# tyiannak/pyAudioAnalysis

Hardware: AMD Instinct MI355X
Metric: short-term frames/sec (34-feat, 16 kHz, 50 ms/25 ms) + HBM GB/s vs peak (higher is better)
Workload: dtype f64

## Files before the change

### include/paa_hip.h

```cpp
#ifndef PAA_HIP_H
#define PAA_HIP_H

#include <stddef.h>
#include <stdint.h>

#ifdef __cplusplus
extern "C" {
#endif

#define PAA_OK                 0
#define PAA_ERR_ARG          (-1)
#define PAA_ERR_UNSUPPORTED  (-2)
#define PAA_ERR_HIP          (-3)
#define PAA_ERR_OOM          (-4)
#define PAA_ERR_TOO_SHORT    (-5)
#define PAA_ERR_CHROMA_VALUE (-6)
#define PAA_ERR_CHROMA_INDEX (-7)
#define PAA_ERR_MEL_INDEX    (-8)
#define PAA_ERR_COMM         (-9)

#define PAA_N_BASE_FEATURES 34

const char *paa_version(void);
const char *paa_last_error(void);
// ... 133 lines not shown
                           const int64_t *offsets, int64_t n_seq, int32_t *d_states, double *d_logprob);
int paa_hmm_dev_loglik_f64(const void *handle, const double *d_feats, int n_dims, int64_t ld, int64_t n_vec, double *d_loglik);
int paa_hmm_train_stats_f64(const double *feats, int n_dims, int64_t ld, int64_t n_vec, const int32_t *labels, int n_states,
                            double *priors, double *transmat, double *means, double *covars);
int paa_hmm_dev_train_stats_f64(const double *d_feats, int n_dims, int64_t ld, int64_t n_vec, const int32_t *labels,
                                int n_states, double *priors, double *transmat, double *means, double *covars);
int paa_debug_hmm_dev_decode_f64(const void *handle, const double *d_feats, int n_dims, int64_t ld, int64_t n_vec,
                                 const int64_t *offsets, int64_t n_seq, int32_t *d_states, double *d_logprob,
                                 int64_t block_rows);

int paa_diar_dev_standardize_f64(const double *d_feats, int n_dims, int64_t ld, int64_t n_vec, double *d_z, double *stats);
int paa_diar_dev_select_rows_f64(const double *d_z, int n_dims, int64_t ld, int64_t n_vec, const int32_t *rows, int n_rows,
                                 double *d_out);
int paa_diar_dev_dim_distances_f64(const double *d_z, int n_dims, int64_t ld, int64_t n_vec, const int32_t *d_labels,
                                   const int32_t *ks, int nk, double *colsum, double *pair_mean);
int paa_diar_dev_sqdist_points_f64(const double *d_z, int n_dims, int64_t ld, int64_t n_vec, const int64_t *idx, int n_pts,
                                   double *out);
int paa_diar_dev_get_points_f64(const double *d_z, int n_dims, int64_t ld, int64_t n_vec, const int64_t *idx, int n_pts,
                                double *out);
int paa_diar_dev_kmeans_f64(const double *d_z, int n_dims, int64_t ld, int64_t n_vec, const int32_t *ks, int nk, double *centers,
                            double tol, int max_iter, int32_t *d_labels, int32_t *n_iter, double *inertia);
int paa_diar_dev_pair_sums_f64(const double *d_z, int n_dims, int64_t ld, int64_t n_vec, const int32_t *d_labels,
                               const int32_t *ks, int nk, double *sums);

int paa_lda_dev_class_stats_f64(const double *d_x, int n_dims, int64_t ld, int64_t n_vec, const int64_t *run_offsets,
                                int64_t n_classes, double *means, double *within_std);
int paa_lda_dev_within_gram_f64(const double *d_x, int n_dims, int64_t ld, int64_t n_vec, const int64_t *run_offsets,
                                int64_t n_classes, const double *means, const double *within_std, double fac, double *gram);
int paa_lda_dev_project_f64(const double *d_x, int n_dims, int64_t ld, int64_t n_vec, const double *xbar, const double *scalings,
                            int n_out, double *d_y, int64_t ld_y);

#define PAA_COMM_ID_BYTES 128
int paa_comm_unique_id(void *id_out );
int paa_comm_init(int world_size, int rank, const void *id);
int paa_comm_destroy(void);
int paa_comm_gather_f64(const double *d_send, const int64_t *counts, int root, double *d_recv);
int paa_comm_gatherv_f64(const double *d_send, const int64_t *counts, const int64_t *displs, int root, double *d_recv);
int paa_comm_barrier(void);

int paa_debug_mel_bank(double fs, int num_fft, double *out_dense);
int paa_debug_dct(double *out_13x40);
int paa_debug_chroma(double fs, int num_fft, int capacity, int32_t *src, double *weight, int32_t *slot);
int paa_debug_wave_trace(uint64_t *out, int max_waves);
int paa_debug_lane_peak(void);
int paa_debug_phase_cycles(uint64_t *out16);
int paa_debug_fft_plan(int window, int32_t *radices, int32_t *fft_len);
int paa_debug_comm_marker_name(const void *unique_id, int rank, char *out, int capacity);
int paa_debug_tri_plan(int window, double fs, int32_t *shape8, int32_t *offsets6, unsigned char *blob, int capacity);
int paa_debug_wg_plan(int window, int32_t *info32, uint16_t *perm, int perm_capacity);
int paa_debug_wgs_plan(int window, int32_t *info16, int32_t *bin_of, int capacity);
int paa_debug_wgr_tables(double fs, int window, int32_t *mel_job, int32_t *mel_fil, int32_t *ch_n, int32_t *ch_src, double *ch_w);
int paa_debug_wgr_runs(const int64_t *frames, int64_t n_clips, int num_cu, int32_t *runs3, int64_t capacity, int64_t *n_runs);
int paa_debug_blu_plan(int window, double fs, int32_t *info8, int32_t *offsets3, unsigned char *blob, int capacity);
int paa_debug_lane_jobs(const int32_t *first, const int32_t *wfirst, const int32_t *cnt, int n_owners, int32_t *jobs256);
int paa_debug_mix_plan(int window, int32_t *radices, int32_t *fft_len, uint16_t *perm, int perm_capacity,
                       int32_t *waves, int32_t *tw_global);
int paa_debug_run_plan(const int64_t *frames, int64_t n_clips, int quantum, int min_run, int max_run, int halo, int wg_runs,
                       int num_cu, int32_t *run_cap, int64_t *n_runs, int32_t *longest);
int paa_debug_run_plan_shrink(const int64_t *frames, int64_t n_clips, int quantum, int min_run, int max_run, int shrink,
                              int wg_runs, int num_cu, int32_t *run_cap, int64_t *n_runs, int32_t *longest);
int64_t paa_debug_balanced_runs(const int64_t *frames, int64_t n_clips, int run_cap, int quantum, int shrink, int wg_runs,
                                int num_cu, int min_run, int32_t *lens, int64_t capacity);

#ifdef __cplusplus
}
#endif
#endif
```

### pyaudioanalysis_amd/_ffi.py

```python
import ctypes as C
import os
import threading

import numpy as np

from . import _build

PAA_OK = 0
ERR_ARG, ERR_UNSUPPORTED, ERR_HIP, ERR_OOM = -1, -2, -3, -4
ERR_TOO_SHORT, ERR_CHROMA_VALUE, ERR_CHROMA_INDEX, ERR_MEL_INDEX, ERR_COMM = -5, -6, -7, -8, -9
COMM_ID_BYTES = 128

_lock = threading.Lock()
_lib = None

c_i16p = C.POINTER(C.c_int16)
c_f64p = C.POINTER(C.c_double)
c_i64p = C.POINTER(C.c_int64)
c_i32p = C.POINTER(C.c_int32)


class HipLibraryError(RuntimeError):
    """libpaa_hip.so is missing / unbuildable, or the HIP runtime reported an error."""

# ... 86 lines not shown
    "paa_forest_destroy": (C.c_int, [C.c_void_p]),
    "paa_forest_num_classes": (C.c_int, [C.c_void_p]),
    "paa_forest_predict_f64": (C.c_int, [C.c_void_p, c_f64p, C.c_int, C.c_int64, C.c_int64, c_f64p, c_f64p, c_i32p, c_f64p,
                                         c_f64p]),
    "paa_forest_dev_predict_f64": (C.c_int, [C.c_void_p, C.c_void_p, C.c_int, C.c_int64, C.c_int64, C.c_void_p, C.c_void_p,
                                             C.c_void_p, C.c_void_p, C.c_void_p]),
    "paa_hmm_create": (C.c_int, [c_f64p, c_f64p, c_f64p, c_f64p, C.c_int, C.c_int, C.POINTER(C.c_void_p)]),
    "paa_hmm_destroy": (C.c_int, [C.c_void_p]),
    "paa_hmm_num_states": (C.c_int, [C.c_void_p]),
    "paa_hmm_decode_f64": (C.c_int, [C.c_void_p, c_f64p, C.c_int, C.c_int64, C.c_int64, c_i64p, C.c_int64, c_i32p, c_f64p]),
    "paa_hmm_dev_decode_f64": (C.c_int, [C.c_void_p, C.c_void_p, C.c_int, C.c_int64, C.c_int64, c_i64p, C.c_int64, C.c_void_p,
                                         C.c_void_p]),
    "paa_hmm_dev_loglik_f64": (C.c_int, [C.c_void_p, C.c_void_p, C.c_int, C.c_int64, C.c_int64, C.c_void_p]),
    "paa_hmm_train_stats_f64": (C.c_int, [c_f64p, C.c_int, C.c_int64, C.c_int64, c_i32p, C.c_int, c_f64p, c_f64p, c_f64p,
                                          c_f64p]),
    "paa_hmm_dev_train_stats_f64": (C.c_int, [C.c_void_p, C.c_int, C.c_int64, C.c_int64, c_i32p, C.c_int, c_f64p, c_f64p,
                                              c_f64p, c_f64p]),
    "paa_debug_hmm_dev_decode_f64": (C.c_int, [C.c_void_p, C.c_void_p, C.c_int, C.c_int64, C.c_int64, c_i64p, C.c_int64,
                                               C.c_void_p, C.c_void_p, C.c_int64]),
    "paa_diar_dev_standardize_f64": (C.c_int, [C.c_void_p, C.c_int, C.c_int64, C.c_int64, C.c_void_p, c_f64p]),
    "paa_diar_dev_select_rows_f64": (C.c_int, [C.c_void_p, C.c_int, C.c_int64, C.c_int64, c_i32p, C.c_int, C.c_void_p]),
    "paa_diar_dev_dim_distances_f64": (C.c_int, [C.c_void_p, C.c_int, C.c_int64, C.c_int64, C.c_void_p, c_i32p, C.c_int, c_f64p,
                                                 c_f64p]),
    "paa_diar_dev_sqdist_points_f64": (C.c_int, [C.c_void_p, C.c_int, C.c_int64, C.c_int64, c_i64p, C.c_int, c_f64p]),
    "paa_diar_dev_get_points_f64": (C.c_int, [C.c_void_p, C.c_int, C.c_int64, C.c_int64, c_i64p, C.c_int, c_f64p]),
    "paa_diar_dev_kmeans_f64": (C.c_int, [C.c_void_p, C.c_int, C.c_int64, C.c_int64, c_i32p, C.c_int, c_f64p, C.c_double,
                                          C.c_int, C.c_void_p, c_i32p, c_f64p]),
    "paa_diar_dev_pair_sums_f64": (C.c_int, [C.c_void_p, C.c_int, C.c_int64, C.c_int64, C.c_void_p, c_i32p, C.c_int, c_f64p]),
    "paa_lda_dev_class_stats_f64": (C.c_int, [C.c_void_p, C.c_int, C.c_int64, C.c_int64, c_i64p, C.c_int64, c_f64p, c_f64p]),
    "paa_lda_dev_within_gram_f64": (C.c_int, [C.c_void_p, C.c_int, C.c_int64, C.c_int64, c_i64p, C.c_int64, c_f64p, c_f64p,
                                              C.c_double, c_f64p]),
    "paa_lda_dev_project_f64": (C.c_int, [C.c_void_p, C.c_int, C.c_int64, C.c_int64, c_f64p, c_f64p, C.c_int, C.c_void_p,
                                          C.c_int64]),
    "paa_comm_unique_id": (C.c_int, [C.c_void_p]),
    "paa_comm_init": (C.c_int, [C.c_int, C.c_int, C.c_void_p]),
    "paa_comm_destroy": (C.c_int, []),
    "paa_comm_gather_f64": (C.c_int, [C.c_void_p, c_i64p, C.c_int, C.c_void_p]),
    "paa_comm_gatherv_f64": (C.c_int, [C.c_void_p, c_i64p, c_i64p, C.c_int, C.c_void_p]),
    "paa_comm_barrier": (C.c_int, []),
    "paa_debug_mel_bank": (C.c_int, [C.c_double, C.c_int, c_f64p]),
    "paa_debug_dct": (C.c_int, [c_f64p]),
    "paa_debug_chroma": (C.c_int, [C.c_double, C.c_int, C.c_int, c_i32p, c_f64p, c_i32p]),
    "paa_debug_phase_cycles": (C.c_int, [C.POINTER(C.c_uint64)]),
    "paa_debug_wave_trace": (C.c_int, [C.POINTER(C.c_uint64), C.c_int]),
    "paa_debug_lane_peak": (C.c_int, []),
    "paa_debug_fft_plan": (C.c_int, [C.c_int, c_i32p, c_i32p]),
    "paa_debug_comm_marker_name": (C.c_int, [C.c_void_p, C.c_int, C.c_char_p, C.c_int]),
    "paa_debug_tri_plan": (C.c_int, [C.c_int, C.c_double, c_i32p, c_i32p, C.c_void_p, C.c_int]),
    "paa_debug_wg_plan": (C.c_int, [C.c_int, c_i32p, C.POINTER(C.c_uint16), C.c_int]),
    "paa_debug_wgs_plan": (C.c_int, [C.c_int, c_i32p, c_i32p, C.c_int]),
    "paa_debug_wgr_tables": (C.c_int, [C.c_double, C.c_int, c_i32p, c_i32p, c_i32p, c_i32p, c_f64p]),
    "paa_debug_wgr_runs": (C.c_int, [c_i64p, C.c_int64, C.c_int, c_i32p, C.c_int64, c_i64p]),
    "paa_debug_blu_plan": (C.c_int, [C.c_int, C.c_double, c_i32p, c_i32p, C.c_void_p, C.c_int]),
    "paa_debug_lane_jobs": (C.c_int, [c_i32p, c_i32p, c_i32p, C.c_int, c_i32p]),
    "paa_debug_mix_plan": (C.c_int, [C.c_int, c_i32p, c_i32p, C.POINTER(C.c_uint16), C.c_int, c_i32p, c_i32p]),
    "paa_debug_run_plan": (C.c_int, [c_i64p, C.c_int64, C.c_int, C.c_int, C.c_int, C.c_int, C.c_int, C.c_int, c_i32p,
                                     c_i64p, c_i32p]),
    "paa_debug_run_plan_shrink": (C.c_int, [c_i64p, C.c_int64, C.c_int, C.c_int, C.c_int, C.c_int, C.c_int, C.c_int, c_i32p,
                                     c_i64p, c_i32p]),
    "paa_debug_balanced_runs": (C.c_int64, [c_i64p, C.c_int64, C.c_int, C.c_int, C.c_int, C.c_int, C.c_int, C.c_int, c_i32p,
                                            C.c_int64]),
}
EXPORTED_SYMBOLS = tuple(sorted(_SIGNATURES))


def library_path():
    return os.environ.get("PAA_HIP_LIBRARY") or _build.LIB


def lib():
    global _lib
    with _lock:
        if _lib is not None:
            return _lib
        path = library_path()
        if path == _build.LIB and _build.is_stale():
            try:
                _build.hipcc_path()
            except RuntimeError as exc:
                if not os.path.exists(path):
                    raise HipLibraryError(
                        "libpaa_hip.so is not built and cannot be built here (%s). "
                        "pyaudioanalysis_amd has no CPU path." % exc)
            else:
                try:
                    _build.build()
                except Exception as exc:
                    raise HipLibraryError("libpaa_hip.so is older than its sources and the rebuild failed:\n%s" % exc)
        try:
            handle = C.CDLL(path)
        except OSError as exc:
            raise HipLibraryError("cannot load %s: %s" % (path, exc))
        for name, (restype, argtypes) in _SIGNATURES.items():
            try:
                fn = getattr(handle, name)
            except AttributeError:
                raise HipLibraryError("%s does not export %s" % (path, name))
            fn.restype = restype
            fn.argtypes = argtypes
        _lib = handle
        return _lib


def last_error():
    msg = lib().paa_last_error()
    return msg.decode("utf-8", "replace") if msg else ""
# ... 180 lines not shown
```

### pyaudioanalysis_amd/csrc/kernels_fast.hpp

```cpp
#pragma once
#include <algorithm>
#include <vector>

#include "device_common.hpp"
#include "tables.hpp"

namespace paa {

struct FastTables {
    void *d_blob = nullptr;
};
namespace f800 {
struct TabLayout {
    int off_w0, off_k0, off_w1, off_k1, off_w2, off_k2;
    int off_chw, off_chk;
    int off_dct;
    int off_tw2, off_twp;
    int off_sync;
    int melN0, melN1, melN2, chN;
    int mel_clamp;
    double f0, rf0, r_half_fs, f0sq;
    int fixed_lists;
    int pace_mode;
    int total;
};
}
struct FastLaunch {
    int run = 0;
    size_t lds = 0;
    const char *name = "";
    int variant = 0;
    int waves_per_cu = 4;
    f800::TabLayout layout;
};

inline void fast_tables_free(FastTables &t) {
    if (t.d_blob) (void)hipFree(t.d_blob);
    t.d_blob = nullptr;
}

namespace f800 {

constexpr int W = 800, NF = 400, QUAD = 4;
constexpr int RAW_PAD = 8;
constexpr int CHUNK = 40;
constexpr int FV_STRIDE = 34;
typedef short s16x2 __attribute__((ext_vector_type(2)));
constexpr int TW_STRIDE = 13;
constexpr int CH_STRIDE = 12;

template <int S, int NW = 4>
struct Geo {
    static_assert(S % CHUNK == 0 && S % 8 == 0, "step must be a multiple of the 40-sample chunk");
    static constexpr int RAW_N = (QUAD - 1) * S + W;
    static constexpr int NCHUNK = RAW_N / CHUNK;
    static constexpr int CPF = S / CHUNK;
    static constexpr int NPRE = (RAW_N / 8 + 63) / 64;
    static constexpr int PAD = (NW == 8 && S == 800) ? 0 : RAW_PAD;
    static constexpr int RAW_BYTES = (RAW_N + 2 * PAD) * 2;
    static constexpr bool ALIAS = (NW == 8);
    static constexpr int OFF_SPEC = 0;
    static constexpr int OFF_RAW = OFF_SPEC + 5 * NF * 8;
    static constexpr int OFF_CE = ALIAS ? OFF_RAW : OFF_RAW + RAW_BYTES;
    static constexpr int OFF_CZ = OFF_CE + NCHUNK * 8;
    static constexpr int OFF_FV = OFF_CZ + 2 * NCHUNK * 4;
    static constexpr int LDS_BYTES = ALIAS ? OFF_FV : OFF_FV + QUAD * FV_STRIDE * 8;
    static constexpr int WAVE_BYTES = ((LDS_BYTES + 15) / 16) * 16;
    static_assert(OFF_RAW % 16 == 0 && OFF_CE % 8 == 0 && OFF_FV % 8 == 0, "LDS alignment");
    static_assert(QUAD * 40 * 8 <= RAW_BYTES, "msp alias fits in the raw buffer");
    static_assert(!ALIAS || RAW_BYTES <= 2 * NF * 8, "raw[] fits in two spectrum slots");
    static_assert(!ALIAS || QUAD * 40 * 8 + QUAD * FV_STRIDE * 8 <= NF * 8, "msp + fv fit in one spectrum slot");
};

__device__ __forceinline__ void dft5r(double2 &a0, double2 &a1, double2 &a2, double2 &a3, double2 &a4) {
    const double c1 = 0.30901699437494742410;
    const double s1 = 0.95105651629515357212, s2 = 0.58778525229247312917;
    const double2 t1 = cadd(a1, a4), t2 = cadd(a2, a3), t3 = csub(a1, a4), t4 = csub(a2, a3);
    const double2 d = csub(t1, t2);
    const double2 h1 = make_double2(fma(-0.5, t1.x, a0.x), fma(-0.5, t1.y, a0.y));
    const double2 h2 = make_double2(fma(-0.5, t2.x, a0.x), fma(-0.5, t2.y, a0.y));
    const double2 m1 = make_double2(fma(c1, d.x, h2.x), fma(c1, d.y, h2.y));
    const double2 m2 = make_double2(fma(-c1, d.x, h1.x), fma(-c1, d.y, h1.y));
    const double2 n1 = make_double2(fma(s2, t4.x, s1 * t3.x), fma(s2, t4.y, s1 * t3.y));
    const double2 n2 = make_double2(fma(-s1, t4.x, s2 * t3.x), fma(-s1, t4.y, s2 * t3.y));
    a0 = make_double2(a0.x + t1.x + t2.x, a0.y + t1.y + t2.y);
    a1 = sub_i(m1, n1);
    a4 = add_i(m1, n1);
    a2 = sub_i(m2, n2);
    a3 = add_i(m2, n2);
}
__device__ __forceinline__ void dft4r(double2 &a0, double2 &a1, double2 &a2, double2 &a3) {
    const double2 t0 = cadd(a0, a2), t1 = csub(a0, a2), t2 = cadd(a1, a3), t3 = csub(a1, a3);
    a0 = cadd(t0, t2);
    a2 = csub(t0, t2);
    a1 = sub_i(t1, t3);
    a3 = add_i(t1, t3);
}
template <int SERIAL>
__device__ __forceinline__ void dft25_tail(double2 *v);
template <int SERIAL = 0>
__device__ __forceinline__ void dft25(double2 *v) {
#pragma unroll
// ... 630 lines not shown

        PAA_TICK(5)
        const double r = (mx == 0.0) ? 1.0 / kEps : fast_div(1.0, mx);
        const double den = sX * r + kEps;
        const double rden = fast_div(1.0, den);
        const double cen = (sIX * r) * rden;
        const double rX = fast_div(1.0, sXe);
        double rXp = rows_from_prev(rX, rX_carry);
        if (first_quad) rXp = (g == 0) ? rX : rXp;
        rX_carry = readlane63(rX);
        const double cb = base_k - cen * rf0;
        double sFa = 0.0, sFb = 0.0;
#pragma unroll
        for (int m = 0; m < 24; m += 2) {
            const double f0d = Xc[m] * rX - Xv[m] * rXp, f1d = Xc[m + 1] * rX - Xv[m + 1] * rXp;
            sFa = fma(f0d, f0d, sFa);
            sFb = fma(f1d, f1d, sFb);
        }
        {
            const double f0d = Xc[24] * rX - Xv[24] * rXp;
            sFa = fma(f0d, f0d, sFa);
        }
        const double sSl = fma(cb, fma(cb, sXl, 2.0 * sMl), sQa + sQb);
        double sSp = sSl * (f0sq * r), sFl = sFa + sFb;
        sSp = group_sum(sSp);
        sFl = group_sum(sFl);
        const double spread = fast_sqrt(sSp * rden);

        int below;
        {
            const double thr = 0.90 * sP;
            const double base = run_incl - cs;
            const double s1 = base + c5[0], s2 = base + pc2, s3 = base + pc3, s4 = base + pc4;
            const bool n0 = !(s1 + kEps > thr), n1 = !(s2 + kEps > thr), n2 = !(s3 + kEps > thr), n3 = !(s4 + kEps > thr);
            const bool n4 = !(run_incl + kEps > thr);
            const int nb = (int)n0 + (int)n1 + (int)n2 + (int)n3 + (int)n4;
            const unsigned long long m1 = __ballot(nb >= 1), m2 = __ballot(nb >= 2), m3 = __ballot(nb >= 3), m4 = __ballot(nb >= 4);
            double run = sel64(m4, s4, sel64(m3, s3, sel64(m2, s2, sel64(m1, s1, base))));
            int in = 0;
#pragma unroll
            for (int u = 0; u < 5; ++u) {
                const double x = sel64(m4, Xc[20 + u], sel64(m3, Xc[15 + u], sel64(m2, Xc[10 + u], sel64(m1, Xc[5 + u], Xc[u]))));
                run = fma(x, x, run);
                in += (run + kEps > thr) ? 0 : 1;
            }
            below = (nb >= 5) ? 25 : 5 * nb + min(in, 4);
        }
        const int first = group_min_i((below < 25) ? 25 * i + below : 0x7fffffff);

        PAA_TICK(6)
        double *mg = msp + 40 * g;
        {
            double acc0 = 0.0, acc1 = 0.0, acc2 = 0.0;
            const int lo0 = t_melk0[i], lo1 = t_melk1[i], lo2 = t_melk2[i];
#define PAA_MEL_CLASS(acc, lo, N, tw, IDX, UNROLL)                                                      \
            UNROLL for (int n = 0; n < (N); n += 8) {                                                   \
                double xv_[8], wv_[8];                                                                  \
                _Pragma("unroll") for (int u = 0; u < 8; ++u) {                                         \
                    xv_[u] = cur[IDX((lo) + n + u)];                                                    \
                    wv_[u] = (tw)[(n + u) * 16 + i];                                                    \
                }                                                                                       \
                double ea_ = 0.0, eb_ = 0.0;                                                            \
                _Pragma("unroll") for (int u = 0; u < 8; u += 2) {                                      \
                    ea_ = fma(xv_[u], wv_[u], ea_);                                                     \
                    eb_ = fma(xv_[u + 1], wv_[u + 1], eb_);                                             \
                }                                                                                       \
                acc += ea_ + eb_;                                                                       \
            }
#define PAA_IDX_CLAMP(k) min((k), NF - 1)
#define PAA_IDX_PLAIN(k) (k)
            if (FIXED) {
                PAA_MEL_CLASS(acc0, lo0, 8, t_melw0, PAA_IDX_PLAIN, _Pragma("unroll"))
                PAA_MEL_CLASS(acc1, lo1, 16, t_melw1, PAA_IDX_PLAIN, _Pragma("unroll"))
                PAA_MEL_CLASS(acc2, lo2, 16, t_melw2, PAA_IDX_PLAIN, _Pragma("unroll"))
            } else if (L.mel_clamp) {
                PAA_MEL_CLASS(acc0, lo0, L.melN0, t_melw0, PAA_IDX_CLAMP, )
                PAA_MEL_CLASS(acc1, lo1, L.melN1, t_melw1, PAA_IDX_CLAMP, )
                PAA_MEL_CLASS(acc2, lo2, L.melN2, t_melw2, PAA_IDX_CLAMP, )
            } else {
                PAA_MEL_CLASS(acc0, lo0, L.melN0, t_melw0, PAA_IDX_PLAIN, )
                PAA_MEL_CLASS(acc1, lo1, L.melN1, t_melw1, PAA_IDX_PLAIN, )
                PAA_MEL_CLASS(acc2, lo2, L.melN2, t_melw2, PAA_IDX_PLAIN, )
            }
#undef PAA_IDX_CLAMP
#undef PAA_IDX_PLAIN
#undef PAA_MEL_CLASS
            acc2 += dpp_mov<0x128>(acc2);
            mg[i] = fast_log10(acc0 + kEps);
            mg[16 + i] = fast_log10(acc1 + kEps);
            const double l2 = fast_log10(acc2 + kEps);
            if (i < 8) mg[32 + i] = l2;
        }
        PAA_TICK(7)
        double chroma = 0.0;
        {
            const int ch_len = FIXED ? 8 : L.chN;
            for (int n = 0; n < ch_len; n += 8) {
                int kv[8];
                double wv[8], xv[8];
#pragma unroll
                for (int u = 0; u < 8; ++u) { kv[u] = t_chk[(n + u) * CH_STRIDE + ich]; wv[u] = t_chw[(n + u) * CH_STRIDE + ich]; }
#pragma unroll
                for (int u = 0; u < 8; ++u) xv[u] = cur[kv[u]];
#pragma unroll
                for (int u = 0; u < 8; ++u) chroma = fma(xv[u] * xv[u], wv[u], chroma);
            }
            chroma = (sP == 0.0) ? chroma / kEps : fast_div(chroma, sP);
            if (i >= 12) chroma = 0.0;
        }
        wsync();
        PAA_TICK(8)
        double *fg = fv + FV_STRIDE * g;
        if (i < 13) {
            const double *dm = t_dct + 41 * i;
            double c0 = 0.0, c1 = 0.0, c2 = 0.0, c3 = 0.0;
#pragma unroll
            for (int h = 0; h < 2; ++h) {
                double dv[20], mv[20];
#pragma unroll
                for (int n = 0; n < 20; ++n) { dv[n] = dm[20 * h + n]; mv[n] = mg[20 * h + n]; }
#pragma unroll
                for (int n = 0; n < 20; n += 4) {
                    c0 = fma(dv[n], mv[n], c0);
                    c1 = fma(dv[n + 1], mv[n + 1], c1);
                    c2 = fma(dv[n + 2], mv[n + 2], c2);
                    c3 = fma(dv[n + 3], mv[n + 3], c3);
                }
            }
            fg[8 + i] = (c0 + c1) + (c2 + c3);
        }
        if (i < 12) fg[21 + i] = chroma;
        if (i == 15) {
            fg[0] = ((double)zc * 0.5) * (1.0 / (double)(W - 1));
            fg[1] = e_tot * (1.0 / (double)W);
            fg[2] = ent_e;
            fg[3] = cen * r_half_fs;
            fg[4] = spread * r_half_fs;
            fg[5] = ent_f;
            fg[6] = (t == 0) ? 0.0 : sFl;
            fg[7] = (first == 0x7fffffff) ? 0.0 : (double)first * (1.0 / (double)NF);
        }
        {
            const double m = group_sum((i < 12) ? chroma : 0.0) / 12.0;
            const double d = (i < 12) ? chroma - m : 0.0;
            const double var = group_sum(d * d) / 12.0;
            if (i == 14) fg[33] = fast_sqrt(var);
        }
        wsync();

        PAA_TICK(9)
        if (lane < kBase) {
            double vq[QUAD];
#pragma unroll
            for (int s = 0; s < QUAD; ++s) vq[s] = fv[FV_STRIDE * s + lane];
            const bool last_quad = q0 + QUAD >= t_end;
            store_row_chunked(oc + (long long)lane * Tc, q0, r0, t_end, last_quad, hold, vq, P.debug);
            if (DELTAS) {
                const double dq[QUAD] = {(q0 == 0) ? 0.0 : vq[0] - vlast, vq[1] - vq[0], vq[2] - vq[1], vq[3] - vq[2]};
                store_row_chunked(oc + (long long)(kBase + lane) * Tc, q0, r0, t_end, last_quad, holdd, dq, P.debug);
#pragma unroll
                for (int j = 0; j < 7; ++j) holdd[j] = (j < 3) ? holdd[j + 4] : dq[j - 3];
            }
#pragma unroll
            for (int j = 0; j < 7; ++j) hold[j] = (j < 3) ? hold[j + 4] : vq[j - 3];
            vlast = vq[QUAD - 1];
        }
        wsync();
        PAA_TICK(10)
    }
    if (NW == 8 && lane == 0) pace[8 + wave] = 0x7fffffff;
    PAA_TEND()
}

}

inline int fast_select(int window, int step, int sample_kind, double fs, FastTables &ft, const FftPlan &fft,
                       const MelTable &mel, const ChromaTable &chroma, FastLaunch &fl, int want_waves) {
    if (!(window == 800 && (step == 400 || step == 800) && sample_kind == 0)) return 0;
    int nw = (want_waves == 8) ? 8 : 4;
    int wave_bytes = (step == 400) ? (nw == 8 ? f800::Geo<400, 8>::WAVE_BYTES : f800::Geo<400, 4>::WAVE_BYTES)
                                   : (nw == 8 ? f800::Geo<800, 8>::WAVE_BYTES : f800::Geo<800, 4>::WAVE_BYTES);
    f800::TabLayout &L = fl.layout;
    auto up4 = [](int n) { return std::max(8, (n + 7) / 8 * 8); };
    int c0 = 0, c1 = 0, c2 = 0, cc = 0;
    for (int m = 0; m < 16; ++m) c0 = std::max(c0, (int)mel.cnt[m]);
    for (int m = 16; m < 32; ++m) c1 = std::max(c1, (int)mel.cnt[m]);
    for (int m = 32; m < 40; ++m) c2 = std::max(c2, ((int)mel.cnt[m] + 1) / 2);
    for (int c = 0; c < 12; ++c) cc = std::max(cc, (int)(chroma.class_start[c + 1] - chroma.class_start[c]));
    L.melN0 = up4(c0); L.melN1 = up4(c1); L.melN2 = up4(c2); L.chN = up4(cc);
    L.mel_clamp = 0;
    for (int i = 0; i < 16; ++i) {
        const int f2 = 32 + (i & 7), half = (mel.cnt[f2] + 1) / 2;
        const int lo2 = mel.lo[f2] + ((i < 8) ? 0 : half);
        if (mel.lo[i] + L.melN0 > f800::NF || mel.lo[16 + i] + L.melN1 > f800::NF || lo2 + L.melN2 > f800::NF) L.mel_clamp = 1;
    }
    L.fixed_lists = (L.melN0 == 8 && L.melN1 == 16 && L.melN2 == 16 && L.chN == 8 && !L.mel_clamp) ? 1 : 0;
    int off = 0;
    auto take = [&off](int bytes) { const int o = off; off += (bytes + 15) / 16 * 16; return o; };
    L.off_w0 = take(L.melN0 * 16 * 8); L.off_k0 = take(16 * 4);
    L.off_w1 = take(L.melN1 * 16 * 8); L.off_k1 = take(16 * 4);
    L.off_w2 = take(L.melN2 * 16 * 8); L.off_k2 = take(16 * 4);
    L.off_chw = take(L.chN * f800::CH_STRIDE * 8);  L.off_chk = take(L.chN * f800::CH_STRIDE * 4);
    L.off_dct = take(13 * 41 * 8);
    L.off_tw2 = take(16 * f800::TW_STRIDE * 16);
    L.off_twp = take(16 * f800::TW_STRIDE * 16);
    L.off_sync = take(16 * 4);
    L.total = off;
    {
        const char *pm = experiment_env("PAA_F800_PACE");
        L.pace_mode = (pm && pm[0] == '0') ? 0 : 1;
    }
    L.f0 = fs / (2.0 * (double)f800::NF);
    L.rf0 = 1.0 / L.f0;
    L.r_half_fs = 1.0 / (fs / 2.0);
    L.f0sq = L.f0 * L.f0;
#ifdef PAA_EXPERIMENTS
    if (nw == 8 && (size_t)L.total + (size_t)nw * wave_bytes > 160 * 1024) {
        nw = 4;
        wave_bytes = (step == 400) ? f800::Geo<400, 4>::WAVE_BYTES : f800::Geo<800, 4>::WAVE_BYTES;
    }
#else
    if (nw != 8) return 0;
#endif
    if ((size_t)L.total + (size_t)nw * wave_bytes > 160 * 1024) return 0;
    if (!ft.d_blob) {
        std::vector<unsigned char> blob((size_t)L.total, 0);
        auto W = [&](int o) { return reinterpret_cast<double *>(blob.data() + o); };
        auto K = [&](int o) { return reinterpret_cast<int32_t *>(blob.data() + o); };
        for (int i = 0; i < 16; ++i) {
            const int f0 = i, f1 = 16 + i, f2 = 32 + (i & 7);
            K(L.off_k0)[i] = mel.lo[f0];
            K(L.off_k1)[i] = mel.lo[f1];
            for (int n = 0; n < mel.cnt[f0]; ++n) W(L.off_w0)[n * 16 + i] = mel.w[mel.off[f0] + n];
            for (int n = 0; n < mel.cnt[f1]; ++n) W(L.off_w1)[n * 16 + i] = mel.w[mel.off[f1] + n];
            const int half = (mel.cnt[f2] + 1) / 2;
            const int b = (i < 8) ? 0 : half, e = (i < 8) ? half : mel.cnt[f2];
            K(L.off_k2)[i] = mel.lo[f2] + b;
            for (int n = b; n < e; ++n) W(L.off_w2)[(n - b) * 16 + i] = mel.w[mel.off[f2] + n];
            if (i < 12)
                for (int n = chroma.class_start[i]; n < chroma.class_start[i + 1]; ++n) {
                    W(L.off_chw)[(n - chroma.class_start[i]) * f800::CH_STRIDE + i] = chroma.w[n];
                    K(L.off_chk)[(n - chroma.class_start[i]) * f800::CH_STRIDE + i] = chroma.src[n];
                }
        }
        double dct[kNumMfcc * kNumMel];
        build_dct(dct);
        for (int q = 0; q < 13; ++q)
            for (int n = 0; n < 40; ++n) W(L.off_dct)[q * 41 + n] = dct[q * 40 + n];
        for (int p = 0; p < f800::TW_STRIDE; ++p)
            for (int r = 0; r < 16; ++r) {
                const int m2 = r * p, mp = p + 25 * r;
                W(L.off_tw2)[2 * (r * f800::TW_STRIDE + p)] = fft.tw[2 * m2];
                W(L.off_tw2)[2 * (r * f800::TW_STRIDE + p) + 1] = fft.tw[2 * m2 + 1];
                W(L.off_twp)[2 * (r * f800::TW_STRIDE + p)] = fft.post[2 * mp];
                W(L.off_twp)[2 * (r * f800::TW_STRIDE + p) + 1] = fft.post[2 * mp + 1];
            }
        if (hipMalloc(&ft.d_blob, blob.size()) != hipSuccess) return PAA_ERR_OOM;
        if (hipMemcpy(ft.d_blob, blob.data(), blob.size(), hipMemcpyHostToDevice) != hipSuccess) return PAA_ERR_HIP;
    }
    fl.name = (step == 400) ? (nw == 8 ? "st_fast_800_w8" : "st_fast_800") : (nw == 8 ? "st_fast_800_s800_w8" : "st_fast_800_s800");
    fl.lds = (size_t)L.total + (size_t)nw * wave_bytes;
    fl.variant = (step == 400) ? 800 : 1600;
    fl.run = 256;
    fl.waves_per_cu = nw;
    return 1;
}

}
```

### pyaudioanalysis_amd/csrc/lib_debug.hpp

```cpp
#pragma once
extern "C" int paa_debug_phase_cycles(uint64_t *out16) {
    if (!out16) return fail(PAA_ERR_ARG, "null");
    for (int i = 0; i < 16; ++i) out16[i] = 0;
#if defined(PAA_F800_TIMING) || defined(PAA_F800_TRACE)
    int rc = ensure_init();
    if (rc) return rc;
    HIP_TRY(hipStreamSynchronize(cs()));
    unsigned long long acc[16] = {0};
    if (launch::phase_fast(acc, nullptr, 0) < 0 || launch::phase_ct(acc, nullptr, 0) < 0 || launch::phase_tri_a(acc, nullptr, 0) < 0 ||
        launch::phase_tri_b(acc, nullptr, 0) < 0 || launch::phase_tri_c(acc, nullptr, 0) < 0 || launch::phase_rmg(acc, nullptr, 0) < 0 || launch::phase_blu(acc, nullptr, 0) < 0 ||
        launch::phase_wgr(acc, nullptr, 0) < 0)
        return fail(PAA_ERR_HIP, "reading the phase counters failed");
    for (int i = 0; i < 16; ++i) out16[i] = acc[i];
#endif
    return PAA_OK;
}

extern "C" int paa_debug_lane_peak(void) {
    std::lock_guard<std::mutex> lk(g_lane_mu);
    const int p = g_lanes_peak;
    g_lanes_peak = g_lanes_active;
    return p;
}

// ... 93 lines not shown
    int64_t n = 0;
    for (const auto &l : out)
        for (int v : l) {
            if (n >= capacity) return fail(PAA_ERR_ARG, "capacity %lld too small", (long long)capacity);
            lens[n++] = v;
        }
    return n;
}
extern "C" int paa_debug_mix_plan(int window, int32_t *radices, int32_t *fft_len, uint16_t *perm, int perm_capacity,
                                  int32_t *waves, int32_t *tw_global) {
    if (window < 2 || !radices || !fft_len) return fail(PAA_ERR_ARG, "bad argument");
    FftPlan p;
    build_fft_plan(window, p);
    *fft_len = p.len;
    mix::MixLayout L;
    if (!mix::mix_layout(p, nullptr, nullptr, 34, L, nullptr)) return 0;
    std::vector<int> radix(L.radix, L.radix + L.n_pass);
    for (int i = 0; i < L.n_pass; ++i) radices[i] = L.radix[i];
    if (perm && perm_capacity >= p.len) {
        std::vector<unsigned short> pm;
        mix::mix_permutation(p.len, radix, pm);
        memcpy(perm, pm.data(), (size_t)p.len * 2);
    }
    if (waves) *waves = L.waves;
    if (tw_global) *tw_global = L.tw_global;
    return L.n_pass;
}
extern "C" int paa_debug_wgr_tables(double fs, int window, int32_t *mel_job, int32_t *mel_fil, int32_t *ch_n, int32_t *ch_src, double *ch_w) {
    const int id = wgr::wgr_shape_id(window);
    if (!id) return 0;
    MelTable mel;
    ChromaTable chroma;
    if (build_mel(fs, window / 2, mel) != PAA_OK || build_chroma(fs, window / 2, chroma) != PAA_OK) return -1;
    std::unique_ptr<wgr::WgrTab> t(new wgr::WgrTab());
    if (!wgr::wgr_build_tab(wgr::wgr_threads(id), &mel, &chroma, *t)) return -1;
    if (mel_job) memcpy(mel_job, t->mel_job, sizeof(t->mel_job));
    if (mel_fil) memcpy(mel_fil, t->mel_fil, sizeof(t->mel_fil));
    if (ch_n) memcpy(ch_n, t->ch_n, sizeof(t->ch_n));
    if (ch_src) memcpy(ch_src, t->ch_src, sizeof(t->ch_src));
    if (ch_w) memcpy(ch_w, t->ch_w, sizeof(t->ch_w));
    return id;
}
extern "C" int paa_debug_wgr_runs(const int64_t *frames, int64_t n_clips, int num_cu, int32_t *runs3, int64_t capacity, int64_t *n_runs) {
    if (!frames || n_clips < 0 || num_cu < 1 || !n_runs) return fail(PAA_ERR_ARG, "bad arguments");
    std::vector<ClipDev> clips((size_t)n_clips);
    for (int64_t c = 0; c < n_clips; ++c) { memset(&clips[(size_t)c], 0, sizeof(ClipDev)); clips[(size_t)c].T = (int)frames[c]; }
    std::vector<Tile> runs;
    wgr::wgr_build_runs(clips, num_cu, runs);
    *n_runs = (int64_t)runs.size();
    for (size_t i = 0; i < runs.size() && (int64_t)i < capacity && runs3; ++i) {
        runs3[3 * i] = runs[i].clip; runs3[3 * i + 1] = runs[i].t0; runs3[3 * i + 2] = runs[i].cnt;
    }
    return PAA_OK;
}

extern "C" int paa_debug_wg_plan(int window, int32_t *info32, uint16_t *perm, int perm_capacity) {
    if (window < 2 || !info32) return fail(PAA_ERR_ARG, "bad argument");
    FftPlan p;
    build_fft_plan(window, p);
    wg::WgLayout L;
    std::vector<unsigned short> pm;
    if (!wg::wg_layout(p, L, pm)) return 0;
    memset(info32, 0, 48 * sizeof(int32_t));
    info32[0] = p.len; info32[1] = window / 2; info32[2] = L.n_pass; info32[3] = L.r0; info32[4] = L.r0 ? L.sub : p.len;
    info32[5] = L.top; info32[6] = L.threads; info32[7] = L.lds_bytes; info32[8] = L.perm_lds; info32[9] = L.feat_staged;
    info32[10] = L.feat_lds_bytes;
    for (int i = 0; i < L.n_pass && i < 12; ++i) { info32[11 + 3 * i] = L.radix[i]; info32[12 + 3 * i] = L.span[i]; info32[13 + 3 * i] = L.tws[i]; }
    if (perm) {
        if (perm_capacity < info32[4]) return fail(PAA_ERR_ARG, "perm capacity %d < %d", perm_capacity, info32[4]);
        memcpy(perm, pm.data(), (size_t)info32[4] * 2);
    }
    return 1;
}
extern "C" int paa_debug_wgs_plan(int window, int32_t *info16, int32_t *bin_of, int capacity) {
    if (window < 2 || !info16) return fail(PAA_ERR_ARG, "bad argument");
    const wgs::Sel sel = wgs::wgs_select(window);
    const int r0 = sel.r0, q = sel.q;
    if (!r0) return 0;
    memset(info16, 0, 16 * sizeof(int32_t));
    const int nf = window / 2;
    const bool a = q == wgs::S3675::Q;
    info16[0] = r0; info16[1] = q;
    info16[2] = a ? wgs::S3675::R1 : wgs::S4000::R1; info16[3] = a ? wgs::S3675::R2 : wgs::S4000::R2; info16[4] = a ? wgs::S3675::R3 : wgs::S4000::R3;
    info16[5] = a ? wgs::S3675::A : wgs::S4000::A; info16[6] = a ? wgs::S3675::NT : wgs::S4000::NT;
    info16[7] = a ? wgs::S3675::LDS_BYTES : wgs::S4000::LDS_BYTES; info16[8] = wgs::wgs_task_types(r0);
    info16[9] = wgs::LCAP;
    info16[10] = a ? (r0 == 12 ? wgs::feat_lds<12, wgs::S3675::Q>() : wgs::feat_lds<6, wgs::S3675::Q>())
                   : (r0 == 12 ? wgs::feat_lds<12, wgs::S4000::Q>() : (r0 == 8 ? wgs::feat_lds<8, wgs::S4000::Q>() : wgs::feat_lds<6, wgs::S4000::Q>()));
    info16[11] = (nf + 64 * r0 - 1) / (64 * r0); info16[12] = wgs::kFeatT;
    info16[13] = a ? (wgs::S3675::P2K0 ? 1 : 0) : (wgs::S4000::P2K0 ? 1 : 0);
    if (bin_of) {
        if (capacity < nf) return fail(PAA_ERR_ARG, "capacity %d < %d", capacity, nf);
        const int h0 = r0 / 2;
        for (int idx = 0; idx < nf; ++idx) {
            const int u = idx / q, kap = idx % q, mm = (u + 1) + r0 * kap;
            bin_of[idx] = (u == h0 - 1) ? h0 * kap : (mm < nf ? mm : window - mm);
        }
    }
    return 1;
}
extern "C" int paa_debug_blu_plan(int window, double fs, int32_t *info8, int32_t *offsets3, unsigned char *blob, int capacity) {
    if (window < 2 || !info8 || !offsets3) return fail(PAA_ERR_ARG, "bad argument");
    (void)fs;
    FftPlan p;
    build_fft_plan(window, p);
    blu::BluLayout L;
// ... 48 lines not shown
```

Baseline: 565.3 million.

## Bin-pack mel filters into lane groups to shrink padded mel dot-product trips

The fast 800-sample kernel's mel stage assigned filters to three 16-lane groups by fixed index, which padded each group to the longest filter. It now sorts filters by length, splits the eight longest across lane pairs and bin-packs them so each group's padded trip count shrinks (fixed case 12/8/4 instead of 8/16/16). The bin and output slot are encoded in the per-lane key, with a pair flag that drives a DPP merge of split halves. This adds a conditional cross-lane add and scattered writes, and falls back to the old grouping if packing fails. A debug export for the tables is also added.

```diff
diff --git a/include/paa_hip.h b/include/paa_hip.h
--- a/include/paa_hip.h
+++ b/include/paa_hip.h
@@ -209,6 +209,7 @@
 int paa_debug_wgr_tables(double fs, int window, int32_t *mel_job, int32_t *mel_fil, int32_t *ch_n, int32_t *ch_src, double *ch_w);
 int paa_debug_wgr_runs(const int64_t *frames, int64_t n_clips, int num_cu, int32_t *runs3, int64_t capacity, int64_t *n_runs);
 int paa_debug_blu_plan(int window, double fs, int32_t *info8, int32_t *offsets3, unsigned char *blob, int capacity);
+int paa_debug_fast800_tables(double fs, int32_t *info24, unsigned char *blob, int capacity);
 int paa_debug_lane_jobs(const int32_t *first, const int32_t *wfirst, const int32_t *cnt, int n_owners, int32_t *jobs256);
 int paa_debug_mix_plan(int window, int32_t *radices, int32_t *fft_len, uint16_t *perm, int perm_capacity,
                        int32_t *waves, int32_t *tw_global);
diff --git a/pyaudioanalysis_amd/_ffi.py b/pyaudioanalysis_amd/_ffi.py
--- a/pyaudioanalysis_amd/_ffi.py
+++ b/pyaudioanalysis_amd/_ffi.py
@@ -162,6 +162,7 @@
     "paa_debug_wgr_tables": (C.c_int, [C.c_double, C.c_int, c_i32p, c_i32p, c_i32p, c_i32p, c_f64p]),
     "paa_debug_wgr_runs": (C.c_int, [c_i64p, C.c_int64, C.c_int, c_i32p, C.c_int64, c_i64p]),
     "paa_debug_blu_plan": (C.c_int, [C.c_int, C.c_double, c_i32p, c_i32p, C.c_void_p, C.c_int]),
+    "paa_debug_fast800_tables": (C.c_int, [C.c_double, c_i32p, C.c_void_p, C.c_int]),
     "paa_debug_lane_jobs": (C.c_int, [c_i32p, c_i32p, c_i32p, C.c_int, c_i32p]),
     "paa_debug_mix_plan": (C.c_int, [C.c_int, c_i32p, c_i32p, C.POINTER(C.c_uint16), C.c_int, c_i32p, c_i32p]),
     "paa_debug_run_plan": (C.c_int, [c_i64p, C.c_int64, C.c_int, C.c_int, C.c_int, C.c_int, C.c_int, C.c_int, c_i32p,
diff --git a/pyaudioanalysis_amd/csrc/kernels_fast.hpp b/pyaudioanalysis_amd/csrc/kernels_fast.hpp
--- a/pyaudioanalysis_amd/csrc/kernels_fast.hpp
+++ b/pyaudioanalysis_amd/csrc/kernels_fast.hpp
@@ -48,6 +48,7 @@
 typedef short s16x2 __attribute__((ext_vector_type(2)));
 constexpr int TW_STRIDE = 13;
 constexpr int CH_STRIDE = 12;
+constexpr int MEL_N0 = 12, MEL_N1 = 8, MEL_N2 = 4;
 
 template <int S, int NW = 4>
 struct Geo {
@@ -784,44 +785,50 @@
         double *mg = msp + 40 * g;
         {
             double acc0 = 0.0, acc1 = 0.0, acc2 = 0.0;
-            const int lo0 = t_melk0[i], lo1 = t_melk1[i], lo2 = t_melk2[i];
-#define PAA_MEL_CLASS(acc, lo, N, tw, IDX, UNROLL)                                                      \
-            UNROLL for (int n = 0; n < (N); n += 8) {                                                   \
-                double xv_[8], wv_[8];                                                                  \
-                _Pragma("unroll") for (int u = 0; u < 8; ++u) {                                         \
-                    xv_[u] = cur[IDX((lo) + n + u)];                                                    \
-                    wv_[u] = (tw)[(n + u) * 16 + i];                                                    \
+            const int kf0 = t_melk0[i], kf1 = t_melk1[i], kf2 = t_melk2[i];
+            const int lo0 = kf0 & 0x7fff, lo1 = kf1 & 0x7fff, lo2 = kf2 & 0x7fff;
+#define PAA_MEL_TRIP(acc, lo, n0, T, tw, IDX)                                                           \
+            {                                                                                           \
+                double xv_[T], wv_[T];                                                                  \
+                _Pragma("unroll") for (int u = 0; u < (T); ++u) {                                       \
+                    xv_[u] = cur[IDX((lo) + (n0) + u)];                                                 \
+                    wv_[u] = (tw)[((n0) + u) * 16 + i];                                                 \
                 }                                                                                       \
                 double ea_ = 0.0, eb_ = 0.0;                                                            \
-                _Pragma("unroll") for (int u = 0; u < 8; u += 2) {                                      \
+                _Pragma("unroll") for (int u = 0; u < (T); u += 2) {                                    \
                     ea_ = fma(xv_[u], wv_[u], ea_);                                                     \
                     eb_ = fma(xv_[u + 1], wv_[u + 1], eb_);                                             \
                 }                                                                                       \
                 acc += ea_ + eb_;                                                                       \
             }
+#define PAA_MEL_GROUP(acc, lo, N, tw, IDX) for (int n = 0; n < (N); n += 4) PAA_MEL_TRIP(acc, lo, n, 4, tw, IDX)
 #define PAA_IDX_CLAMP(k) min((k), NF - 1)
 #define PAA_IDX_PLAIN(k) (k)
             if (FIXED) {
-                PAA_MEL_CLASS(acc0, lo0, 8, t_melw0, PAA_IDX_PLAIN, _Pragma("unroll"))
-                PAA_MEL_CLASS(acc1, lo1, 16, t_melw1, PAA_IDX_PLAIN, _Pragma("unroll"))
-                PAA_MEL_CLASS(acc2, lo2, 16, t_melw2, PAA_IDX_PLAIN, _Pragma("unroll"))
+                static_assert(MEL_N0 == 12 && MEL_N1 == 8 && MEL_N2 == 4, "trip sizes below");
+                PAA_MEL_TRIP(acc0, lo0, 0, 6, t_melw0, PAA_IDX_PLAIN)
+                PAA_MEL_TRIP(acc0, lo0, 6, 6, t_melw0, PAA_IDX_PLAIN)
+                PAA_MEL_TRIP(acc1, lo1, 0, 8, t_melw1, PAA_IDX_PLAIN)
+                PAA_MEL_TRIP(acc2, lo2, 0, 4, t_melw2, PAA_IDX_PLAIN)
             } else if (L.mel_clamp) {
-                PAA_MEL_CLASS(acc0, lo0, L.melN0, t_melw0, PAA_IDX_CLAMP, )
-                PAA_MEL_CLASS(acc1, lo1, L.melN1, t_melw1, PAA_IDX_CLAMP, )
-                PAA_MEL_CLASS(acc2, lo2, L.melN2, t_melw2, PAA_IDX_CLAMP, )
+                PAA_MEL_GROUP(acc0, lo0, L.melN0, t_melw0, PAA_IDX_CLAMP)
+                PAA_MEL_GROUP(acc1, lo1, L.melN1, t_melw1, PAA_IDX_CLAMP)
+                PAA_MEL_GROUP(acc2, lo2, L.melN2, t_melw2, PAA_IDX_CLAMP)
             } else {
-                PAA_MEL_CLASS(acc0, lo0, L.melN0, t_melw0, PAA_IDX_PLAIN, )
-                PAA_MEL_CLASS(acc1, lo1, L.melN1, t_melw1, PAA_IDX_PLAIN, )
-                PAA_MEL_CLASS(acc2, lo2, L.melN2, t_melw2, PAA_IDX_PLAIN, )
+                PAA_MEL_GROUP(acc0, lo0, L.melN0, t_melw0, PAA_IDX_PLAIN)
+                PAA_MEL_GROUP(acc1, lo1, L.melN1, t_melw1, PAA_IDX_PLAIN)
+                PAA_MEL_GROUP(acc2, lo2, L.melN2, t_melw2, PAA_IDX_PLAIN)
             }
 #undef PAA_IDX_CLAMP
 #undef PAA_IDX_PLAIN
-#undef PAA_MEL_CLASS
-            acc2 += dpp_mov<0x128>(acc2);
-            mg[i] = fast_log10(acc0 + kEps);
-            mg[16 + i] = fast_log10(acc1 + kEps);
-            const double l2 = fast_log10(acc2 + kEps);
-            if (i < 8) mg[32 + i] = l2;
+#undef PAA_MEL_GROUP
+#undef PAA_MEL_TRIP
+            acc0 += (kf0 & 0x8000) ? dpp_mov<0x128>(acc0) : 0.0;
+            acc1 += (kf1 & 0x8000) ? dpp_mov<0x128>(acc1) : 0.0;
+            acc2 += (kf2 & 0x8000) ? dpp_mov<0x128>(acc2) : 0.0;
+            mg[kf0 >> 16] = fast_log10(acc0 + kEps);
+            mg[kf1 >> 16] = fast_log10(acc1 + kEps);
+            mg[kf2 >> 16] = fast_log10(acc2 + kEps);
         }
         PAA_TICK(7)
         double chroma = 0.0;
@@ -906,6 +913,121 @@
 
 }
 
+namespace f800 {
+struct MelCell { int filter, b, e; };
+inline void mel_cells(const MelTable &mel, MelCell (&cell)[3][16], unsigned (&pair)[3]) {
+    struct Item { int size, filter, split; };
+    std::vector<int> by_cnt(kNumMel);
+    for (int m = 0; m < kNumMel; ++m) by_cnt[m] = m;
+    std::stable_sort(by_cnt.begin(), by_cnt.end(), [&](int x, int y) { return mel.cnt[x] != mel.cnt[y] ? mel.cnt[x] > mel.cnt[y] : x > y; });
+    std::vector<Item> items;
+    for (int r = 0; r < kNumMel; ++r) {
+        const int m = by_cnt[r], split = r < 8 ? 1 : 0;
+        items.push_back({split ? (mel.cnt[m] + 1) / 2 : (int)mel.cnt[m], m, split});
+    }
+    std::stable_sort(items.begin(), items.end(), [](const Item &x, const Item &y) { return x.size != y.size ? x.size > y.size : x.filter < y.filter; });
+    std::vector<Item> in_group[3];
+    int free_cells[3] = {16, 16, 16};
+    bool ok = true;
+    for (const Item &it : items) {
+        int g = 0;
+        while (g < 3 && free_cells[g] < 1 + it.split) ++g;
+        if (g == 3) { ok = false; break; }
+        in_group[g].push_back(it);
+        free_cells[g] -= 1 + it.split;
+    }
+    if (!ok) {
+        for (int g = 0; g < 3; ++g) in_group[g].clear();
+        for (int m = 0; m < 32; ++m) in_group[m / 16].push_back({(int)mel.cnt[m], m, 0});
+        for (int m = 32; m < kNumMel; ++m) in_group[2].push_back({((int)mel.cnt[m] + 1) / 2, m, 1});
+    }
+    for (int g = 0; g < 3; ++g) {
+        int p = 0;
+        bool used[16] = {false};
+        pair[g] = 0;
+        for (const Item &it : in_group[g])
+            if (it.split) {
+                const int half = (mel.cnt[it.filter] + 1) / 2;
+                cell[g][p] = {it.filter, 0, half};
+                cell[g][p + 8] = {it.filter, half, (int)mel.cnt[it.filter]};
+                used[p] = used[p + 8] = true;
+                pair[g] |= (1u << p) | (1u << (p + 8));
+                ++p;
+            }
+        int lane = 0;
+        for (const Item &it : in_group[g])
+            if (!it.split) {
+                while (used[lane]) ++lane;
+                cell[g][lane] = {it.filter, 0, (int)mel.cnt[it.filter]};
+                used[lane] = true;
+            }
+    }
+}
+
+inline void build_tables(double fs, const FftPlan &fft, const MelTable &mel, const ChromaTable &chroma, TabLayout &L,
+                         std::vector<unsigned char> *blob) {
+    MelCell cell[3][16];
+    unsigned pair[3];
+    mel_cells(mel, cell, pair);
+    int len[3] = {0, 0, 0}, cc = 0;
+    for (int g = 0; g < 3; ++g)
+        for (int i = 0; i < 16; ++i) len[g] = std::max(len[g], cell[g][i].e - cell[g][i].b);
+    for (int c = 0; c < 12; ++c) cc = std::max(cc, (int)(chroma.class_start[c + 1] - chroma.class_start[c]));
+    auto up4 = [](int n) { return std::max(4, (n + 3) / 4 * 4); };
+    auto up8 = [](int n) { return std::max(8, (n + 7) / 8 * 8); };
+    L.melN0 = up4(len[0]); L.melN1 = up4(len[1]); L.melN2 = up4(len[2]); L.chN = up8(cc);
+    const int N[3] = {L.melN0, L.melN1, L.melN2};
+    L.mel_clamp = 0;
+    for (int g = 0; g < 3; ++g)
+        for (int i = 0; i < 16; ++i)
+            if (mel.lo[cell[g][i].filter] + cell[g][i].b + N[g] > NF) L.mel_clamp = 1;
+    L.fixed_lists = (L.melN0 == MEL_N0 && L.melN1 == MEL_N1 && L.melN2 == MEL_N2 && L.chN == 8 && !L.mel_clamp) ? 1 : 0;
+    int off = 0;
+    auto take = [&off](int bytes) { const int o = off; off += (bytes + 15) / 16 * 16; return o; };
+    L.off_w0 = take(L.melN0 * 16 * 8); L.off_k0 = take(16 * 4);
+    L.off_w1 = take(L.melN1 * 16 * 8); L.off_k1 = take(16 * 4);
+    L.off_w2 = take(L.melN2 * 16 * 8); L.off_k2 = take(16 * 4);
+    L.off_chw = take(L.chN * CH_STRIDE * 8);  L.off_chk = take(L.chN * CH_STRIDE * 4);
+    L.off_dct = take(13 * 41 * 8);
+    L.off_tw2 = take(16 * TW_STRIDE * 16);
+    L.off_twp = take(16 * TW_STRIDE * 16);
+    L.off_sync = take(16 * 4);
+    L.total = off;
+    L.f0 = fs / (2.0 * (double)NF);
+    L.rf0 = 1.0 / L.f0;
+    L.r_half_fs = 1.0 / (fs / 2.0);
+    L.f0sq = L.f0 * L.f0;
+    if (!blob) return;
+    blob->assign((size_t)L.total, 0);
+    auto W = [&](int o) { return reinterpret_cast<double *>(blob->data() + o); };
+    auto K = [&](int o) { return reinterpret_cast<int32_t *>(blob->data() + o); };
+    const int off_w[3] = {L.off_w0, L.off_w1, L.off_w2}, off_k[3] = {L.off_k0, L.off_k1, L.off_k2};
+    for (int g = 0; g < 3; ++g)
+        for (int i = 0; i < 16; ++i) {
+            const MelCell &c = cell[g][i];
+            K(off_k[g])[i] = (mel.lo[c.filter] + c.b) | (((pair[g] >> i) & 1u) ? 0x8000 : 0) | (c.filter << 16);
+            for (int n = c.b; n < c.e; ++n) W(off_w[g])[(n - c.b) * 16 + i] = mel.w[mel.off[c.filter] + n];
+        }
+    for (int i = 0; i < 12; ++i)
+        for (int n = chroma.class_start[i]; n < chroma.class_start[i + 1]; ++n) {
+            W(L.off_chw)[(n - chroma.class_start[i]) * CH_STRIDE + i] = chroma.w[n];
+            K(L.off_chk)[(n - chroma.class_start[i]) * CH_STRIDE + i] = chroma.src[n];
+        }
+    double dct[kNumMfcc * kNumMel];
+    build_dct(dct);
+    for (int q = 0; q < 13; ++q)
+        for (int n = 0; n < 40; ++n) W(L.off_dct)[q * 41 + n] = dct[q * 40 + n];
+    for (int p = 0; p < TW_STRIDE; ++p)
+        for (int r = 0; r < 16; ++r) {
+            const int m2 = r * p, mp = p + 25 * r;
+            W(L.off_tw2)[2 * (r * TW_STRIDE + p)] = fft.tw[2 * m2];
+            W(L.off_tw2)[2 * (r * TW_STRIDE + p) + 1] = fft.tw[2 * m2 + 1];
+            W(L.off_twp)[2 * (r * TW_STRIDE + p)] = fft.post[2 * mp];
+            W(L.off_twp)[2 * (r * TW_STRIDE + p) + 1] = fft.post[2 * mp + 1];
+        }
+}
+}
+
 inline int fast_select(int window, int step, int sample_kind, double fs, FastTables &ft, const FftPlan &fft,
                        const MelTable &mel, const ChromaTable &chroma, FastLaunch &fl, int want_waves) {
     if (!(window == 800 && (step == 400 || step == 800) && sample_kind == 0)) return 0;
@@ -913,39 +1035,11 @@
     int wave_bytes = (step == 400) ? (nw == 8 ? f800::Geo<400, 8>::WAVE_BYTES : f800::Geo<400, 4>::WAVE_BYTES)
                                    : (nw == 8 ? f800::Geo<800, 8>::WAVE_BYTES : f800::Geo<800, 4>::WAVE_BYTES);
     f800::TabLayout &L = fl.layout;
-    auto up4 = [](int n) { return std::max(8, (n + 7) / 8 * 8); };
-    int c0 = 0, c1 = 0, c2 = 0, cc = 0;
-    for (int m = 0; m < 16; ++m) c0 = std::max(c0, (int)mel.cnt[m]);
-    for (int m = 16; m < 32; ++m) c1 = std::max(c1, (int)mel.cnt[m]);
-    for (int m = 32; m < 40; ++m) c2 = std::max(c2, ((int)mel.cnt[m] + 1) / 2);
-    for (int c = 0; c < 12; ++c) cc = std::max(cc, (int)(chroma.class_start[c + 1] - chroma.class_start[c]));
-    L.melN0 = up4(c0); L.melN1 = up4(c1); L.melN2 = up4(c2); L.chN = up4(cc);
-    L.mel_clamp = 0;
-    for (int i = 0; i < 16; ++i) {
-        const int f2 = 32 + (i & 7), half = (mel.cnt[f2] + 1) / 2;
-        const int lo2 = mel.lo[f2] + ((i < 8) ? 0 : half);
-        if (mel.lo[i] + L.melN0 > f800::NF || mel.lo[16 + i] + L.melN1 > f800::NF || lo2 + L.melN2 > f800::NF) L.mel_clamp = 1;
-    }
-    L.fixed_lists = (L.melN0 == 8 && L.melN1 == 16 && L.melN2 == 16 && L.chN == 8 && !L.mel_clamp) ? 1 : 0;
-    int off = 0;
-    auto take = [&off](int bytes) { const int o = off; off += (bytes + 15) / 16 * 16; return o; };
-    L.off_w0 = take(L.melN0 * 16 * 8); L.off_k0 = take(16 * 4);
-    L.off_w1 = take(L.melN1 * 16 * 8); L.off_k1 = take(16 * 4);
-    L.off_w2 = take(L.melN2 * 16 * 8); L.off_k2 = take(16 * 4);
-    L.off_chw = take(L.chN * f800::CH_STRIDE * 8);  L.off_chk = take(L.chN * f800::CH_STRIDE * 4);
-    L.off_dct = take(13 * 41 * 8);
-    L.off_tw2 = take(16 * f800::TW_STRIDE * 16);
-    L.off_twp = take(16 * f800::TW_STRIDE * 16);
-    L.off_sync = take(16 * 4);
-    L.total = off;
+    f800::build_tables(fs, fft, mel, chroma, L, nullptr);
     {
         const char *pm = experiment_env("PAA_F800_PACE");
         L.pace_mode = (pm && pm[0] == '0') ? 0 : 1;
     }
-    L.f0 = fs / (2.0 * (double)f800::NF);
-    L.rf0 = 1.0 / L.f0;
-    L.r_half_fs = 1.0 / (fs / 2.0);
-    L.f0sq = L.f0 * L.f0;
 #ifdef PAA_EXPERIMENTS
     if (nw == 8 && (size_t)L.total + (size_t)nw * wave_bytes > 160 * 1024) {
         nw = 4;
@@ -956,37 +1050,8 @@
 #endif
     if ((size_t)L.total + (size_t)nw * wave_bytes > 160 * 1024) return 0;
     if (!ft.d_blob) {
-        std::vector<unsigned char> blob((size_t)L.total, 0);
-        auto W = [&](int o) { return reinterpret_cast<double *>(blob.data() + o); };
-        auto K = [&](int o) { return reinterpret_cast<int32_t *>(blob.data() + o); };
-        for (int i = 0; i < 16; ++i) {
-            const int f0 = i, f1 = 16 + i, f2 = 32 + (i & 7);
-            K(L.off_k0)[i] = mel.lo[f0];
-            K(L.off_k1)[i] = mel.lo[f1];
-            for (int n = 0; n < mel.cnt[f0]; ++n) W(L.off_w0)[n * 16 + i] = mel.w[mel.off[f0] + n];
-            for (int n = 0; n < mel.cnt[f1]; ++n) W(L.off_w1)[n * 16 + i] = mel.w[mel.off[f1] + n];
-            const int half = (mel.cnt[f2] + 1) / 2;
-            const int b = (i < 8) ? 0 : half, e = (i < 8) ? half : mel.cnt[f2];
-            K(L.off_k2)[i] = mel.lo[f2] + b;
-            for (int n = b; n < e; ++n) W(L.off_w2)[(n - b) * 16 + i] = mel.w[mel.off[f2] + n];
-            if (i < 12)
-                for (int n = chroma.class_start[i]; n < chroma.class_start[i + 1]; ++n) {
-                    W(L.off_chw)[(n - chroma.class_start[i]) * f800::CH_STRIDE + i] = chroma.w[n];
-                    K(L.off_chk)[(n - chroma.class_start[i]) * f800::CH_STRIDE + i] = chroma.src[n];
-                }
-        }
-        double dct[kNumMfcc * kNumMel];
-        build_dct(dct);
-        for (int q = 0; q < 13; ++q)
-            for (int n = 0; n < 40; ++n) W(L.off_dct)[q * 41 + n] = dct[q * 40 + n];
-        for (int p = 0; p < f800::TW_STRIDE; ++p)
-            for (int r = 0; r < 16; ++r) {
-                const int m2 = r * p, mp = p + 25 * r;
-                W(L.off_tw2)[2 * (r * f800::TW_STRIDE + p)] = fft.tw[2 * m2];
-                W(L.off_tw2)[2 * (r * f800::TW_STRIDE + p) + 1] = fft.tw[2 * m2 + 1];
-                W(L.off_twp)[2 * (r * f800::TW_STRIDE + p)] = fft.post[2 * mp];
-                W(L.off_twp)[2 * (r * f800::TW_STRIDE + p) + 1] = fft.post[2 * mp + 1];
-            }
+        std::vector<unsigned char> blob;
+        f800::build_tables(fs, fft, mel, chroma, L, &blob);
         if (hipMalloc(&ft.d_blob, blob.size()) != hipSuccess) return PAA_ERR_OOM;
         if (hipMemcpy(ft.d_blob, blob.data(), blob.size(), hipMemcpyHostToDevice) != hipSuccess) return PAA_ERR_HIP;
     }
diff --git a/pyaudioanalysis_amd/csrc/lib_debug.hpp b/pyaudioanalysis_amd/csrc/lib_debug.hpp
--- a/pyaudioanalysis_amd/csrc/lib_debug.hpp
+++ b/pyaudioanalysis_amd/csrc/lib_debug.hpp
@@ -169,6 +169,30 @@
         runs3[3 * i] = runs[i].clip; runs3[3 * i + 1] = runs[i].t0; runs3[3 * i + 2] = runs[i].cnt;
     }
     return PAA_OK;
+}
+
+extern "C" int paa_debug_fast800_tables(double fs, int32_t *info24, unsigned char *blob, int capacity) {
+    if (!info24 || !(fs > 0.0)) return fail(PAA_ERR_ARG, "bad argument");
+    MelTable mel;
+    ChromaTable chroma;
+    FftPlan fft;
+    int rc = build_mel(fs, f800::NF, mel);
+    if (rc) return fail(rc, "mel filter bank indexes bin >= num_fft");
+    rc = build_chroma(fs, f800::NF, chroma);
+    if (rc) return fail(rc, "chroma table error");
+    build_fft_plan(f800::W, fft);
+    f800::TabLayout L;
+    std::vector<unsigned char> b;
+    f800::build_tables(fs, fft, mel, chroma, L, &b);
+    const int32_t info[19] = {L.off_w0, L.off_k0, L.off_w1, L.off_k1, L.off_w2, L.off_k2, L.melN0, L.melN1, L.melN2, L.mel_clamp,
+                              L.fixed_lists, 0, 0, 0, L.off_chw, L.off_chk, L.chN, L.off_dct, L.total};
+    memset(info24, 0, 24 * sizeof(int32_t));
+    memcpy(info24, info, sizeof(info));
+    if (blob) {
+        if (capacity < (int)b.size()) return fail(PAA_ERR_ARG, "blob capacity %d < %d", capacity, (int)b.size());
+        memcpy(blob, b.data(), b.size());
+    }
+    return (int)b.size();
 }
 
 extern "C" int paa_debug_wg_plan(int window, int32_t *info32, uint16_t *perm, int perm_capacity) {
```

After: 568.4 million, median of 6. About the same (+0.5%).
